# view-sonic/Cloud-Server

Hardware: AMD Instinct MI355X
Metric: train_samples_per_s (higher is better)
Workload: dtype fp32; 1 GPU; model=reference sample CNN (API.md:306-332), 2,276,218 params, global_batch=50, per_gpu_batch=50, optimizer=AdagradOptimizer, parallelism=dp1, backend=hip, hip_graph=True, collectives=none, xgmi=single rank

## Files before the change

cloud_server_amd/csrc/kernels/dense_direct.hip:

```cpp
#include "common.h"
#include "optim_common.h"
#include "head_dgrad.h"
#include <cstdlib>

namespace csa {

typedef float dd_f32x16 __attribute__((ext_vector_type(16)));

constexpr int DD_THREADS = 256;
constexpr int DD_WAVES = 4;
constexpr int DD_SLAB_ROWS = 16;
constexpr int DD_MAXC = 128;
constexpr int DD_U = 4;

__constant__ long long* g_dd_dbg = nullptr;
#define DD_STAMP(i)                                                                           \
  do {                                                                                        \
    if (g_dd_dbg && threadIdx.x == 0 && blockIdx.x == 0 && blockIdx.y == 0 && blockIdx.z == 0) \
      g_dd_dbg[i] = (long long)__builtin_amdgcn_s_memtime();                                  \
  } while (0)
#define DD_SPAN_BEGIN()                                                                       \
  do {                                                                                        \
    if (g_dd_dbg && threadIdx.x == 0)                                                         \
      atomicMin((unsigned long long*)&g_dd_dbg[4], (unsigned long long)__builtin_amdgcn_s_memtime()); \
  } while (0)
#define DD_SPAN_END()                                                                         \
  do {                                                                                        \
    if (g_dd_dbg && threadIdx.x == 0)                                                         \
      atomicMax((unsigned long long*)&g_dd_dbg[5], (unsigned long long)__builtin_amdgcn_s_memtime()); \
  } while (0)

__device__ __forceinline__ int dd_row(int r, int lane) { return (r & 3) + 8 * (r >> 2) + 4 * (lane >> 5); }

__device__ __forceinline__ void dd_pin4(float4& v) { asm volatile("" : "+v"(v.x), "+v"(v.y), "+v"(v.z), "+v"(v.w)); }
__device__ __forceinline__ void dd_pin(float& v) { asm volatile("" : "+v"(v)); }

__device__ __forceinline__ float dd_c(const float4& v, int s) {
  return s == 0 ? v.x : (s == 1 ? v.y : (s == 2 ? v.z : v.w));
}

struct DDTile { float v[8]; int row[8]; int col[8]; };

__device__ __forceinline__ DDTile dd_reduce(float* s_red, const dd_f32x16& a0, const dd_f32x16& a1) {
  const int t = threadIdx.x, lane = t & 63, w = t >> 6;
#pragma unroll
  for (int r = 0; r < 16; ++r) {
    s_red[(w * 32 + r) * 64 + lane] = a0[r];
    s_red[(w * 32 + 16 + r) * 64 + lane] = a1[r];
  }
  __syncthreads();
  DDTile out;
#pragma unroll
  for (int q = 0; q < 8; ++q) {
    const int idx = t + q * DD_THREADS;
    const int v = idx >> 6, ln = idx & 63;
    float s = s_red[(0 * 32 + v) * 64 + ln];
#pragma unroll
    for (int ww = 1; ww < DD_WAVES; ++ww) s += s_red[(ww * 32 + v) * 64 + ln];
    out.v[q] = s;
    out.row[q] = (v >> 4) * 32 + dd_row(v & 15, ln);
    out.col[q] = ln & 31;
  }
  return out;
}

__device__ __forceinline__ void dd_wave_range(int k0, int k1, int& a, int& b) {
  const int w = threadIdx.x >> 6;
  const int n8 = (k1 - k0 + 7) >> 3;
  const int per = (n8 + DD_WAVES - 1) / DD_WAVES;
  a = min(k1, k0 + w * per * 8);
  b = min(k1, a + per * 8);
}

struct DDFwd {
  const float* x; const float* w; const float* bias; float* y;
  int M, N, K, act; float alpha; int ksplit, kper;
  int life_base;
};

__constant__ long long* g_dd_life = nullptr;


template <bool V4>
__device__ __forceinline__ void dd_fwd_body(const DDFwd& a, const int nt, const int mb, const int ks, float* s_red);
// ... 384 lines not shown
      const int m = min(c0 + 2 * s + h, a.M - 1);
      xa[s] = a.x[(long)m * a.F + f];
      ya[s] = a.dy[(long)m * a.N + nc];
    }
#pragma unroll
    for (int s = 0; s < DD_KC; ++s) {
      dd_pin(xa[s]);
      dd_pin(ya[s]);
    }
#pragma unroll
    for (int s = 0; s < DD_KC; ++s) {
      if (c0 + 2 * s >= a.M) break;
      const float ok = c0 + 2 * s + h < a.M ? 1.f : 0.f;
      float xv = a.act != ACT_NONE ? act_fwd(xa[s], a.act, a.alpha) : xa[s];
      acc = __builtin_amdgcn_mfma_f32_32x32x2f32(xv * ok, ya[s], acc, 0, 0, 0);
    }
  }
  DD_STAMP(1);
  if (!upd) {
#pragma unroll
    for (int r = 0; r < 16; ++r) {
      const int ff = f0 + dd_row(r, lane);
      if (ff < a.F && nn < a.N) a.dw[(long)ff * a.N + nn] = acc[r] * a.gscale;
    }
    return;
  }
  const float lr = opt_step_lr(a.opt, a.lr, a.step);
#pragma unroll
  for (int r = 0; r < 16; ++r) {
    dd_pin(wv[r]);
    dd_pin(s0[r]);
    dd_pin(s1[r]);
  }
#pragma unroll
  for (int r = 0; r < 16; ++r) {
    const int ff = f0 + dd_row(r, lane);
    if (ff >= a.F || nn >= a.N) continue;
    const long idx = (long)ff * a.N + nn;
    opt_update(a.opt, lr, wv[r], acc[r] * a.gscale, s0[r], s1[r]);
    a.w[idx] = wv[r];
    if (ns > 0) a.sw0[idx] = s0[r];
    if (ns > 1) a.sw1[idx] = s1[r];
  }
  DD_STAMP(3);
  DD_SPAN_END();
}

constexpr int DW_WAVES = 16;
constexpr int DW_THREADS = 64 * DW_WAVES;
constexpr size_t DW_LDS = (size_t)DW_WAVES * 16 * 64 * sizeof(float);

struct DWGroup { float4 x[DD_U]; float b[DD_U][4]; };

__global__ __launch_bounds__(DW_THREADS) void dd_fwd_wide_kernel(DDFwd a, int ntile) {
  extern __shared__ __attribute__((aligned(16))) float s_part[];
  DD_STAMP(0);
  DD_SPAN_BEGIN();
  const int lb = (int)blockIdx.x, tid = threadIdx.x;
  if (g_dd_life && tid == 0) g_dd_life[2 * lb + 2 * a.life_base] = (long long)__builtin_amdgcn_s_memrealtime();
  const int lane = tid & 63, i = lane & 31, h = lane >> 5;
  const int wave = __builtin_amdgcn_readfirstlane(tid >> 6);
  const int nt = lb % ntile, ks = (lb / ntile) % a.ksplit, mb = lb / (ntile * a.ksplit);
  const int n0 = nt * 32, m0 = mb * 32;
  const int kg0 = ks * a.kper, kg1 = min(a.K, kg0 + a.kper);
  const int per = (((kg1 - kg0 + 7) >> 3) + DW_WAVES - 1) / DW_WAVES;
  const int ka = min(kg1, kg0 + wave * per * 8), kb = min(kg1, ka + per * 8);
  const float* xr = a.x + (long)min(m0 + i, a.M - 1) * a.K;
  const float* wc = a.w + min(n0 + i, a.N - 1);
  const int er = wave;
  float bias = (a.bias && ks == 0) ? a.bias[min(n0 + i, a.N - 1)] : 0.f;

  auto load = [&](DWGroup& g, int k) {
#pragma unroll
    for (int u = 0; u < DD_U; ++u) {
      if (k + 8 * u >= kb) break;
      const int kk = k + 8 * u + 4 * h;
      g.x[u] = *reinterpret_cast<const float4*>(xr + min(kk, a.K - 4));
#pragma unroll
      for (int s = 0; s < 4; ++s) g.b[u][s] = wc[(long)min(kk + s, a.K - 1) * a.N];
    }
  };
  dd_f32x16 acc = {};
  auto mac = [&](DWGroup& g, int k) {
#pragma unroll
    for (int u = 0; u < DD_U; ++u) {
      if (k + 8 * u >= kb) break;
      dd_pin4(g.x[u]);
#pragma unroll
      for (int s = 0; s < 4; ++s) dd_pin(g.b[u][s]);
      float xv[4] = {g.x[u].x, g.x[u].y, g.x[u].z, g.x[u].w};
      if (a.act != ACT_NONE) {
#pragma unroll
        for (int s = 0; s < 4; ++s) xv[s] = act_fwd(xv[s], a.act, a.alpha);
      }
      const bool in = k + 8 * u + 4 * h < kb;
#pragma unroll
      for (int s = 0; s < 4; ++s)
        acc = __builtin_amdgcn_mfma_f32_32x32x2f32(xv[s], in ? g.b[u][s] : 0.f, acc, 0, 0, 0);
    }
  };
  if (ka < kb) {
    DWGroup cur, nxt;
    load(cur, ka);
    for (int k = ka;; k += 8 * DD_U) {
      if (k + 8 * DD_U < kb) {
        load(nxt, k + 8 * DD_U);
        mac(cur, k);
        cur = nxt;
      } else {
        mac(cur, k);
        break;
      }
    }
  }
  DD_STAMP(1);
  dd_pin(bias);
#pragma unroll
  for (int r = 0; r < 16; ++r) s_part[(wave * 16 + r) * 64 + lane] = acc[r];
  __syncthreads();
  float v = bias;
  {
    const float* src = s_part + er * 64 + lane;
    float s = src[0];
#pragma unroll
    for (int w = 1; w < DW_WAVES; ++w) s += src[w * 16 * 64];
    v += s;
  }
  DD_STAMP(2);
  const int m = m0 + dd_row(er, lane), nn = n0 + i;
  if (m < a.M && nn < a.N) {
    float* p = a.y + (long)m * a.N + nn;
    if (a.ksplit > 1) atomicAdd(p, v); else *p = v;
  }
  if (g_dd_life && tid == 0) g_dd_life[2 * lb + 2 * a.life_base + 1] = (long long)__builtin_amdgcn_s_memrealtime();
  DD_STAMP(3);
  DD_SPAN_END();
}

static int dd_splits(int tiles, int K) {
  if (g_csa_det) return 1;
  static const int target = [] {
    const char* e = std::getenv("CSA_DD_TARGET");
    const int v = e ? std::atoi(e) : 2048;
    return v >= 256 && v <= 16384 ? v : 2048;
  }();
  int ks = (target / DD_WAVES + tiles - 1) / tiles;
  const int maxks = (K + 8 * DD_WAVES * 2 - 1) / (8 * DD_WAVES * 2);
  ks = ks < 1 ? 1 : ks;
  ks = ks > maxks ? maxks : ks;
  return ks < 1 ? 1 : ks;
}

static int dd_kper(int K, int ks) { return (((K + ks - 1) / ks) + 7) & ~7; }

static bool dd_wide(int K) {
  static const int wide_env = [] { const char* e = std::getenv("CSA_DD_WIDE"); return e ? (e[0] == '0' ? 0 : 1) : -1; }();
  if (wide_env == 0 || g_csa_det || g_csa_shared || (g_csa_packed && wide_env != 1)) return false;
  return K % 4 == 0;
}

struct DDPlan { bool wide; int ks, kper; };

static DDPlan dd_fwd_plan(int M, int N, int K) {
  DDPlan p;
  p.wide = dd_wide(K);
  if (p.wide) {
    static const int cap = [] { const char* e = std::getenv("CSA_DD_WIDE_KS"); return e ? std::atoi(e) : 0; }();
    const int tiles = ((N + 31) / 32) * ((M + 31) / 32);
    const int maxks = K / (8 * DW_WAVES);
    p.ks = 256 / tiles;
    p.ks = p.ks > maxks ? maxks : p.ks;
    p.ks = cap > 0 && p.ks > cap ? cap : p.ks;
    p.ks = p.ks < 1 ? 1 : p.ks;
  } else {
    p.ks = dd_splits(((N + 31) / 32) * ((M + 63) / 64), K);
  }
  p.kper = dd_kper(K, p.ks);
  p.ks = (K + p.kper - 1) / p.kper;
  return p;
}

}

using namespace csa;

CSA_API int csa_dd_life_debug(long long* p) {
  return (int)hipMemcpyToSymbol(HIP_SYMBOL(g_dd_life), &p, sizeof(p));
}

// ... 45 lines not shown
CSA_API int csa_chain_head_debug(long long* p) {
  return (int)hipMemcpyToSymbol(HIP_SYMBOL(g_hd_dbg), &p, sizeof(p));
}

static thread_local DDFwdGroup g_dd_group{};
static thread_local bool g_dd_grouping = false;
CSA_API void csa_dd_group_begin() { g_dd_grouping = true; g_dd_group.g = 0; }
CSA_API int csa_dd_group_end(hipStream_t st) {
  g_dd_grouping = false;
  const int G = g_dd_group.g;
  if (G == 0) return 0;
  const DDFwd& a0 = g_dd_group.a[0];
  for (int j = 1; j < G; ++j) {
    const DDFwd& a = g_dd_group.a[j];
    if (a.M != a0.M || a.N != a0.N || a.K != a0.K || a.ksplit != a0.ksplit || a.kper != a0.kper) return -2;
  }
  g_dd_group.ks = a0.ksplit;
  const dim3 grid((a0.N + 31) / 32, (a0.M + 63) / 64, a0.ksplit * G);
  if (a0.K % 4 == 0) hipLaunchKernelGGL(dd_fwd_group_kernel<true>, grid, dim3(DD_THREADS), 0, st, g_dd_group);
  else hipLaunchKernelGGL(dd_fwd_group_kernel<false>, grid, dim3(DD_THREADS), 0, st, g_dd_group);
  g_dd_group.g = 0;
  return (int)hipGetLastError();
}

CSA_API int csa_dd_fwd(const float* X, const float* W, const float* bias, float* Y, int M, int N, int K,
                       int act, float alpha, hipStream_t st) {
  if (M <= 0 || N <= 0 || K <= 0) return -1;
  const int nt = (N + 31) / 32, mb = (M + 63) / 64;
  const DDPlan plan = dd_fwd_plan(M, N, K);
  const int ks = plan.ks, kper = plan.kper;
  DDFwd a{X, W, bias, Y, M, N, K, act, alpha, ks, kper, 0};
  a.life_base = K > 1024 ? 0 : 4096;
  if (g_chain_on) {
    if (g_chain_n >= 2) return -4;
    g_chain_f[g_chain_n++] = a;
    return 0;
  }
  if (g_dd_grouping) {
    if (g_dd_group.g >= DD_GMAX) return -3;
    g_dd_group.a[g_dd_group.g++] = a;
    return 0;
  }
  if (plan.wide) {
    static const bool attr = hipFuncSetAttribute((const void*)dd_fwd_wide_kernel,
                                                 hipFuncAttributeMaxDynamicSharedMemorySize, (int)DW_LDS) == hipSuccess;
    (void)attr;
    const unsigned blocks = (unsigned)(nt * ((M + 31) / 32) * ks);
    hipLaunchKernelGGL(dd_fwd_wide_kernel, dim3(blocks), dim3(DW_THREADS), DW_LDS, st, a, nt);
  } else if (K % 4 == 0) hipLaunchKernelGGL(dd_fwd_kernel<true>, dim3(nt, mb, ks), dim3(DD_THREADS), 0, st, a);
  else hipLaunchKernelGGL(dd_fwd_kernel<false>, dim3(nt, mb, ks), dim3(DD_THREADS), 0, st, a);
  return (int)hipGetLastError();
}

CSA_API int csa_dd_dgrad_splits(int M, int F, int N) {
  return dd_splits(((F + 31) / 32) * ((M + 63) / 64), N);
}

CSA_API int csa_dd_dgrad_slabs() { return DD_SLAB_ROWS; }

CSA_API int csa_dd_dgrad(const float* dY, const float* W, float* dX, int M, int F, int N,
                         const float* x_fwd, int act, float alpha, const float* bn_slab, int bn_nslab, int bn_C,
                         float bn_count, float bn_eps, const float* bn_scale, const float* bn_offset,
                         float* bwd_slab, hipStream_t st) {
  if (M <= 0 || F <= 0 || N <= 0) return -1;
  if (bn_slab && (bn_C > DD_MAXC || bn_C <= 0 || !bwd_slab)) return -1;
  const int ft = (F + 31) / 32, mb = (M + 63) / 64;
  int ks = dd_splits(ft * mb, N);
  const int kper = dd_kper(N, ks);
  ks = (N + kper - 1) / kper;
  DDDgrad a{dY, W, dX, M, F, N, ks, kper, x_fwd, act, alpha,
            BNRef{bn_slab, bn_nslab, bn_C, bn_count, bn_eps, bn_scale, bn_offset}, bwd_slab};
  if (N % 4 == 0) hipLaunchKernelGGL(dd_dgrad_kernel<true>, dim3(ft, mb, ks), dim3(DD_THREADS), 0, st, a);
  else hipLaunchKernelGGL(dd_dgrad_kernel<false>, dim3(ft, mb, ks), dim3(DD_THREADS), 0, st, a);
  return (int)hipGetLastError();
}

CSA_API int csa_dd_wgrad(const float* X, const float* dY, int M, int F, int N, int act, float alpha, float gscale,
                         float* dW, float* db, float* W, float* b, float* sW0, float* sW1, float* sb0, float* sb1,
                         int opt, float lr, const int64_t* step, hipStream_t st) {
  if (M <= 0 || F <= 0 || N <= 0) return -1;
  if (opt < 0 && (!dW || !db)) return -2;
  if (opt >= 0 && (!W || !b || (opt_nslots(opt) > 0 && (!sW0 || !sb0)) || (opt_nslots(opt) > 1 && (!sW1 || !sb1))))
    return -3;
  DDWgrad a{X, dY, M, F, N, act, alpha, gscale, dW, db, W, b, sW0, sW1, sb0, sb1, opt, lr, step,
            (F + 31) / 32, (N + 127) / 128};
  const int nb = a.ftiles * a.ntiles + (N + 63) / 64;
  hipLaunchKernelGGL(dd_wgrad_kernel, dim3(nb), dim3(DD_THREADS), 0, st, a);
  return (int)hipGetLastError();
}
```

cloud_server_amd/ops/fused.py:

```python
from __future__ import annotations

import ctypes as C
import os
from typing import Optional, Sequence

import torch

from . import build as _build

_LIB: Optional[C.CDLL] = None

P = C.c_void_p
I = C.c_int
L = C.c_long
F = C.c_float
U64 = C.c_uint64

ACT_IDS = {None: 0, "none": 0, "sigmoid": 1, "relu": 2, "leaky_relu": 3}

_SIGS = {
    "csa_dense_fwd_splits": (I, [I, I, I]),
    "csa_dense_fwd": (I, [P, P, P, P, I, I, I, P, I, I, F, F, P, P, I, F, P]),
    "csa_dense_dgrad": (I, [P, P, P, I, I, I, P, I, F, P, I, I, F, F, P, P, P, P]),
    "csa_dense_dgrad_splits": (I, [I, I, I, I]),
# ... 62 lines not shown
    "csa_chain_head_debug": (I, [P]),
    "csa_dd_life_debug": (I, [P]),
    "csa_ew_life_debug": (I, [P]),
    "csa_dd_group_end": (I, [P]),
    "csa_cp_du_debug": (I, [P]),
    "csa_conv_pair_bn_tab": (None, [P]),
    "csa_conv_pair_c1_size": (L, [P]),
    "csa_conv_pair_c1_bands": (I, [P, P, I]),
    "csa_conv_pair_c1_fwd": (None, [P, L]),
    "csa_conv_pair_c1_bwd": (None, [P, L]),
    "csa_head_debug": (I, [P]),
    "csa_conv_pair_fwd": (I, [P, P, P, P, P, P, I, F, P, P, I, F, P, P, P, I, P, P, I, P]),
    "csa_conv_pair_fwd_carry": (I, [I, F, P, P, P, P, P, P, I, P, P, I]),
    "csa_opt_carry_flush": (I, [I, F, P, P, P, P, P, P, I, P, P, I, P]),
    "csa_optimizer_set_pending": (None, [P]),
    "csa_dense_update_flush_last": (I, [P]),
    "csa_conv_pair_tail_table_bytes": (L, [P, I]),
    "csa_conv_pair_tail_plan": (I, [P, I, I, P, P, P, P, P, P, P, P, I]),
    "csa_dense_update_grad_mode": (I, [P, P]),
    "csa_conv_pair_tail_set": (I, [P, P, I, F, P, P, I, I, P, P, P, P, P, P, I, L, P, P]),
    "csa_conv_pair_tail_force": (None, [P]),
    "csa_conv_pair_tail_pending": (I, []),
    "csa_conv_pair_tail_ticket_words": (I, []),
    "csa_dense_update_head_params": (I, [P, P, P, P, P, P]),
    "csa_conv_pair_valu_ok": (I, [P]),
    "csa_conv_pair_grid": (I, [P]),
    "csa_set_deterministic": (None, [I]),
    "csa_deterministic": (I, []),
    "csa_set_packed": (None, [I]),
    "csa_packed": (I, []),
    "csa_set_shared_gpu": (None, [I]),
    "csa_shared_gpu": (I, []),
    "csa_rows_fold": (I, [P, L, I, L, P, I, P]),
    "csa_rows_fold_multi": (I, [I, P, P, P, P, P, P, P]),
    "csa_conv_pair_bwd": (I, [P, P, P, P, P, P, I, F, P, I, I, F, P, P, P, P, I, F, F, P, P, P, I, P, P, P, P, F,
                              P, P, P, P, I, P, P]),
    "csa_conv_pair_bwd_tables_size": (L, [P]),
    "csa_conv_pair_bwd_tables": (I, [P, P, P]),
    "csa_conv_pair_bwd_units": (I, [P, I, P, I]),
    "csa_conv_pair_bwd_units_load": (I, [P, I, P]),
    "csa_conv_pair_bwd_bias_mode": (I, [P, I, I]),
    "csa_head_part": (I, [P, I, I, I, F, P, P, P, P, P, I, F, P, P, P, P, P, P, P]),
    "csa_head_part2": (I, [P, I, I, I, F, P, P, P, P, P, I, F, P, P, P, P, P, P, P, L, P]),
    "csa_gather_batch": (I, [P, P, P, P, I, L, P, P, P]),
    "csa_gather_images_f32": (I, [P, P, P, I, L, P, P]),
    "csa_zero": (I, [P, P, I, P]),
    "csa_gemm_debug": (I, [P]),
    "csa_conv_debug": (I, [P]),
    "csa_bn_act_apply": (I, [P, P, L, I, P, I, F, F, P, P, I, F, P, P]),
    "csa_dd_debug": (I, [P]),
    "csa_dd_fwd_splits": (I, [I, I, I]),
    "csa_dd_fwd_wide": (I, [I, I, I]),
    "csa_dd_fwd": (I, [P, P, P, P, I, I, I, I, F, P]),
    "csa_dd_dgrad_splits": (I, [I, I, I]),
    "csa_dd_dgrad_slabs": (I, []),
    "csa_dd_dgrad": (I, [P, P, P, I, I, I, P, I, F, P, I, I, F, F, P, P, P, P]),
    "csa_dd_wgrad": (I, [P, P, I, I, I, I, F, F, P, P, P, P, P, P, P, P, I, F, P, P]),
    "csa_gconv_fwd_splits": (I, [P]),
    "csa_gconv_fwd": (I, [P, P, P, P, P, P]),
    "csa_gconv_wgrad_splits": (I, [P, I]),
    "csa_gconv_wgrad": (I, [P, P, P, P, P, F, P]),
    "csa_gconv_dgrad_splits": (I, [P]),
    "csa_gconv_dgrad": (I, [P, P, P, P, P]),
    "csa_bn_slab_rows": (I, []),
    "csa_bn_stat_rows": (I, [L]),
    "csa_bn_stats": (I, [P, L, I, P, I, P]),
    "csa_bn_finalize": (I, [P, I, I, F, F, P, P, P, P, F, I, P, P]),
    "csa_bn_apply": (I, [P, P, L, I, P, I, F, P]),
    "csa_bn_bwd_reduce": (I, [P, P, P, L, I, P, I, F, P, I, P]),
    "csa_bn_bwd_finalize": (I, [P, I, I, F, F, P, P, P, P]),
    "csa_bn_bwd_apply": (I, [P, P, P, P, L, I, P, P, I, F, P]),
    "csa_maxpool_fwd": (I, [P, P, P, P, P]),
    "csa_maxpool_bwd": (I, [P, P, P, P, P]),
    "csa_drop_fwd": (I, [P, P, L, L, L, L, U64, P, P, I, F, I, F, I, P]),
    "csa_drop_bwd": (I, [P, P, P, L, L, L, L, U64, P, I, F, I, F, P]),
    "csa_xgmi_alloc":(I, [L, C.POINTER(P), P]),
    "csa_xgmi_open": (I, [P, C.POINTER(P)]),
    "csa_xgmi_reuse": (I, [P, L, P]),
    "csa_xgmi_close": (I, [P]),
    "csa_xgmi_free": (I, [P]),
    "csa_xgmi_handle_bytes": (I, []),
    "csa_xgmi_max_blocks": (I, []),
    "csa_xgmi_diag_words": (I, []),
    "csa_xgmi_run": (I, [I, I, I, L, P, P, I, P, P, P, P, C.c_double, I, P, P]),
    "csa_xgmi_reduce_scatter": (I, [I, I, L, P, P, P, L, L, L, P, P, C.c_double, I, P, P]),
    "csa_aps_step": (I, [I, I, I, I, L, I, P, P, P, P, P, P, I, F, P, P, I, C.c_double, P]),
}


def lib_path() -> str:
    return os.environ.get("CSA_KERNEL_LIB") or _build.KERNEL_LIB


def available() -> bool:
    return os.path.exists(lib_path())


def load(required: bool = True) -> Optional[C.CDLL]:
    global _LIB
    if _LIB is not None:
        return _LIB
    path = lib_path()
    if not os.path.exists(path):
        if os.environ.get("CSA_AUTOBUILD", "1") == "1":
            try:
                _build.build_kernels()
# ... 40 lines not shown
```

cloud_server_amd/runtime/hip_program.py:

```python
from __future__ import annotations

import ctypes as C
import ctypes as _ctypes
import os
from dataclasses import dataclass, field
from typing import Dict, List, Optional

import torch

from ..models.dsl import ActSpec, ConvSpec, DenseSpec, DropoutSpec, LayerPlan, NormSpec, PoolSpec
from ..ops import dropout_ref
from ..ops import fused as K
from ..ops import fused as _FK
from ..ops import optim_ref
from ..utils.streams import dedicated_stream


def _opt_call(lib, name: str, *args):
    try:
        fn = getattr(lib, name)
    except AttributeError:
        return None
    return fn(*args)

# ... 70 lines not shown
    norm: Optional[LayerPlan] = None


class HipProgram:
    WGRAD_STRIPES = int(os.environ.get("CSA_WGRAD_STRIPES", "16"))
    FWD_ZERO_MAX = 4

    def __init__(self, eng, forward_only: bool = False):
        self.e = eng
        self.forward_only = forward_only
        self.lib = K.load(required=True)
        _set_nt_out(self.lib)
        if eng.device.type != "cuda":
            raise Unsupported("HIP program needs a GPU device")
        self.det = bool(getattr(eng, "deterministic", False)) and not forward_only
        self.packed = bool(getattr(eng, "packed", False)) and os.environ.get("CSA_PACKED_PROFILE", "1") == "1"
        self.shared_gpu = bool(getattr(eng, "shared_gpu", False))
        with self._det_scope():
            self._init_plan(eng, forward_only)

    def _det_scope(self):
        prog = self

        class _Scope:
            def __enter__(self_):
                self_.prev = (int(prog.lib.csa_deterministic()), int(prog.lib.csa_packed()),
                              int(prog.lib.csa_shared_gpu()))
                prog.lib.csa_set_deterministic(1 if prog.det else 0)
                prog.lib.csa_set_packed(1 if prog.packed else 0)
                prog.lib.csa_set_shared_gpu(1 if prog.shared_gpu else 0)

            def __exit__(self_, *exc):
                prog.lib.csa_set_deterministic(self_.prev[0])
                prog.lib.csa_set_packed(self_.prev[1])
                prog.lib.csa_set_shared_gpu(self_.prev[2])
                return False
        return _Scope()

    def _init_plan(self, eng, forward_only: bool) -> None:
        self.B = eng.cfg.batch_size
        self.model = eng.model
        self.sync_bn = bool(eng.model.sync_bn)
        self.W = eng.ctx.world if self.sync_bn else 1
        self.views = eng.model.state.views(eng.flat)
        self.gviews = {} if forward_only else eng.model.state.views(eng.flat_grad)
        self._lower()
        self._plan_fused()
        self._plan_pair()
        self._plan_hfuse()
        if self.det:
            self._check_det()
        self._alloc()
        self._plan_splits()
        self.pair_tabs = None
        if self.pair is not None and not forward_only:
            n = int(self.lib.csa_conv_pair_bwd_tables_size(K.ints(self.pair)))
            if n > 0:
                self.pair_tabs = torch.zeros(n, dtype=torch.int32, device=eng.device)
                self._rc(self.lib.csa_conv_pair_bwd_tables(K.ints(self.pair), K.ptr(self.pair_tabs), K.stream()),
                         "conv_pair_bwd_tables")
        if forward_only:
            self.staged = False
            return
        self._plan_lowrank()
        self.zero_regions: List[torch.Tensor] = []
        self._collect_zero_regions()
        self._zero_now()
        self._plan_stage()
        self._plan_grad_buckets()
        self._plan_carry()
        self.opt_segments = self._opt_segments()
        self._plan_tail()
        self._plan_chain()

    def _plan_chain(self) -> None:
        e = self.e
        self.chain = False
        try:
            chain_ok = self.lib.csa_chain_ok
        except AttributeError:
            return
        dense = [u for u in self.units if u.kind == "dense"]
        if (e.ctx.enabled or self.det or self.packed or self.forward_only
                or not getattr(self, "head_dgrad", False) or os.environ.get("CSA_FWD_CHAIN", "0") != "1"
                or len(dense) != 2 or self.units[-2:] != dense or not all(u.direct for u in dense)
                or getattr(self, "br_unit", None) is not None
                or not chain_ok(self.units[-1].layer.spec.hidden)):
            return
        self.chain_tk = torch.zeros(int(self.lib.csa_chain_words()), dtype=torch.int32, device=e.device)
        self.chain_err = torch.zeros(1, dtype=torch.int32, device=e.device)
        self.chain = True

    def _plan_carry(self) -> None:
        self.carry = None
        e = self.e
        if (not e.ctx.enabled or e.sync.strategy != "allreduce" or e.aps is not None or self.pair is None
                or os.environ.get("CSA_DP_CARRY", "1") != "1"
                or not self.lib.csa_conv_pair_valu_ok(K.ints(self.pair))):
            return
        offs = self.model.state.offsets
        keep = set(self.keep_ranges)
        n = self.e.flat.numel()
        spans = sorted(offs.values())
        ends = {o: (spans[i + 1] if i + 1 < len(spans) else n) for i, o in enumerate(spans)}
        carried, segs = set(), []
        for u in self.units:
            if u.kind != "dense" or (u.fused and self.fused) or u.lr_update:
                continue
            names = [f"{u.layer.name}.weight", f"{u.layer.name}.bias"]
            if not all((offs[nm], offs[nm] + (self.gviews[nm].numel() // 4) * 4) in keep for nm in names):
                continue
            for nm in names:
                carried.add(offs[nm])
        if not carried:
            return
        for o in spans:
            if o not in carried:
                continue
            lo, hi = o - o % 4, -(-ends[o] // 4) * 4
            if segs and segs[-1][1] >= lo:
                segs[-1][1] = max(segs[-1][1], hi)
            else:
                segs.append([lo, hi])
        if len(segs) > 4:
            return
        m4 = sum(hi - lo for lo, hi in segs) // 4
        self.carry = segs
        self.carry_offsets = carried
        self.carry_blocks = max(1, min(1024, -(-m4 // 256)))
        self.carry_pending = torch.zeros(1, dtype=torch.int32, device=e.device)
        u2 = self.units[2] if len(self.units) > 2 else None
        self.carry_clear = bool(u2 is not None and u2.kind == "dense" and u2.xt is not None)

    def _carry_args(self):
        e = self.e
        s0 = e.slots[0] if e.slots.shape[0] > 0 else None
        s1 = e.slots[1] if e.slots.shape[0] > 1 else None
        lo = (C.c_long * 4)(*[x[0] for x in self.carry])
        hi = (C.c_long * 4)(*[x[1] for x in self.carry])
        return (e.opt_id, float(e.lr), K.ptr(e.dstep), K.ptr(e.flat), K.ptr(e.flat_grad), K.ptr(s0), K.ptr(s1),
                K.ptr(self.carry_pending), len(self.carry), lo, hi, self.carry_blocks)

    def flush(self, st=None) -> None:
        if getattr(self, "carry", None) is None:
# ... 541 lines not shown
                tf.count = float(B * ph * pw * self.W)
                if fo:
                    continue
                C = src.y.shape[3]
                if u.kind == "dense" and u.fused:
                    nb = self.lib.csa_dense_bwd_update_slabs(u.layer.in_shape.numel)
                elif u.kind == "dense":
                    nb = self.lib.csa_dense_dgrad_slabs(B, u.layer.in_shape.numel, u.layer.spec.hidden)
                else:
                    nb = self.lib.csa_conv_dgrad_nslab(self._conv_geom(u.layer, B))
                tf.bwd_slab = torch.zeros(nb, 2, C, **f32)
                tf.bwd_nslab = nb
                if self.det:
                    tf.bwd_prod_rows, tf.bwd_nslab = nb, 1
        for u in self.units:
            u.xt = None
            if u.kind == "dense" and u.in_tf.has_bn and u.layer.in_shape.numel % 4 == 0:
                u.xt = torch.zeros(B, u.layer.in_shape.numel, **f32)
            if u.kind == "dense" and u.fused and not fo:
                ws = (_ctypes.c_longlong * 2)()
                self.lib.csa_dense_bwd_update_ws(u.layer.in_shape.numel, u.layer.spec.hidden, ws)
                u.du_part = torch.zeros(max(int(ws[0]), 1), **f32)
                u.du_cnt = torch.zeros(max(int(ws[1]), 1), dtype=torch.int32, device=dev)
            u.in_tf.bn_tab = torch.zeros(4, u.in_tf.slab.shape[2], **f32) if u.xt is not None else None
        self.dlast = self.units[-1].dy
        if getattr(self, "head_row", False):
            self.hdl = torch.zeros(B, 10, **f32)
            self.hrl = torch.zeros(B, **f32)
            self.hrc = torch.zeros(B, dtype=torch.int32, device=dev)
        self.idx = None
        if self.head_rg:
            K = self.dlast[0].numel()
            G = -(-B // self.head_rg)
            self.head_part = torch.zeros(G, (K * 10 + 10 + 3) // 4 * 4, **f32)
            self.head_kw = K * 10
            self.head_mloss = torch.zeros(G, **f32)
            self.head_mcorr = torch.zeros(G, dtype=torch.int32, device=dev)
        self.pair_c1 = None
        if (self.pair is not None and not fo and not self.det and os.environ.get("CSA_PAIR_C1", "1") == "1"
                and self.lib.csa_conv_pair_valu_ok(_FK.ints(self.pair))):
            n = _opt_call(self.lib, "csa_conv_pair_c1_size", _FK.ints(self.pair))
            if n is not None and int(n) > 0:
                self.pair_c1 = torch.zeros(int(n), **f32)

    def _plan_splits(self) -> None:
        B = self.B
        for u in self.units:
            if u.kind == "dense":
                fin, fout = u.layer.in_shape.numel, u.layer.spec.hidden
                u.splits_fwd = (self.lib.csa_dd_fwd_splits(B, fout, fin) if u.direct
                                else self.lib.csa_dense_fwd_splits(B, fout, fin))
            elif u.kind == "gconv":
                u.splits_fwd = self.lib.csa_gconv_fwd_splits(self._conv_geom(u.layer, B))

    def _collect_zero_regions(self) -> None:
        B = self.B
        regs: List[torch.Tensor] = []
        flat: List[torch.Tensor] = []
        self.stripe_bufs: List[torch.Tensor] = []
        fold_budget = 8 - (2 if self.head_rg else 0)
        for k, u in enumerate(self.units):
            lp = u.layer
            if u.kind == "dense":
                fin, fout = lp.in_shape.numel, lp.spec.hidden
                if u.splits_fwd > 1:
                    regs.append(u.y)
                if u.fused:
                    continue
                if k > 0:
                    tfm = u.in_tf.has_bn or u.in_tf.act is not None
                    if self.lib.csa_dense_dgrad_splits(B, fin, fout, int(tfm)) > 1:
                        regs.append(self.units[k - 1].dy)
                if self.lib.csa_dense_wgrad_splits(B, fin, fout) > 1:
                    flat.append(self.gviews[f"{lp.name}.weight"].view(-1))
                    flat.append(self.gviews[f"{lp.name}.bias"])
            elif u.kind == "gconv":
                geom = self._conv_geom(lp, B)
                if u.splits_fwd > 1:
                    regs.append(u.y.view(-1))
                if k > 0 and self.lib.csa_gconv_dgrad_splits(geom) > 1:
                    regs.append(self.units[k - 1].dy.view(-1))
                if self.lib.csa_gconv_wgrad_splits(geom, int(bool(lp.spec.bias))) > 1:
                    flat.append(self.gviews[f"{lp.name}.weight"].view(-1))
                    if lp.spec.bias:
                        flat.append(self.gviews[f"{lp.name}.bias"])
            elif u.kind == "bn":
                if u.norm is not None:
                    regs += [u.bn_slab.view(-1), u.bn_bslab.view(-1)]
            elif u.kind == "conv":
                nf = 1 + (1 if lp.spec.bias else 0)
                S = 1 if self.e.ctx.enabled or fold_budget < nf else self.WGRAD_STRIPES
                in_pair = self.pair is not None and k < 2
                u.tail_fold = in_pair and getattr(self, "dp_hf", False)
                u.row_fold = self.det or (in_pair and self.e.ctx.enabled and not u.tail_fold)
                if u.tail_fold:
                    S = self.WGRAD_STRIPES
                if u.row_fold:
                    if not self.det:
                        S = self.WGRAD_STRIPES
                    elif in_pair:
                        S = int(self.lib.csa_conv_pair_grid(_FK.ints(self.pair)))
                    else:
                        S = int(self.lib.csa_conv_wgrad_blocks(self._conv_geom(lp, B), int(bool(lp.spec.bias))))
                        if S <= 0:
                            raise Unsupported(f"conv unit {lp.name}: no weight-gradient plan")
                elif S > 1:
# ... 296 lines not shown
                        K.ptr(u.dw_acc), K.ptr(u.db_acc) if sp.bias else None, u.wg_stripes, st), "conv_bwd")
                    self._conv_det_folds(u, tf, st)
                    self._grad_ready(k)
                    continue
                ws = st
                self._rc(lib.csa_conv_wgrad(
                    None if raw else K.ptr(u.x), K.ptr(img) if raw else None, K.ptr(rows) if raw else None,
                    K.ptr(dc), K.ptr(u.dw_acc), K.ptr(u.db_acc) if sp.bias else None, u.wg_stripes,
                    B, h, w, lp.in_shape.c, sp.kh, sp.kw, sp.stride[0], sp.stride[1], lp.pads[0], lp.pads[2],
                    oh, ow, sp.cout, bn[0], bn[1], bn[2], bn[3], bn[4], bn[5], in_act, in_alpha,
                    K.ptr(cur) if raw else None, ws), "conv_wgrad")
                if prev is not None:
                    self._rc(lib.csa_conv_dgrad(
                        K.ptr(dc), K.ptr(V[f"{lp.name}.weight"]), K.ptr(prev.dy), geom,
                        K.ptr(u.x), in_act, in_alpha, *bn, K.ptr(tf.bwd_slab), st), "conv_dgrad")
                self._conv_det_folds(u, tf, st)
            self._grad_ready(k)

        main = torch.cuda.current_stream(e.device)
        if e.aps is not None:
            e.aps.step(e.flat_grad, e.flat, e.slots)
            self._optimizer(st)
            return
        if self.overlap:
            main.wait_stream(self.side)
        elif e.ctx.enabled and e.sync.strategy == "lowrank":
            e.sync.allreduce_ranges(e.flat_grad, self.lr_ranges, tag="lr_rem")
            if self.lr_units:
                main.wait_stream(self.lr_side)
        else:
            e.after_backward_sync()
        if getattr(self, "tail", False):
            if lib.csa_dense_update_pending() or lib.csa_conv_pair_tail_pending():
                raise RuntimeError("pair-backward tail / deferred updates not consumed")
            if self.tail_update:
                return
        self._optimizer(st)

    _eval_bn = False

    def _forward(self, st) -> None:
        e, lib, B = self.e, self.lib, self.B
        rows, cur = e.stream.rows, e.stream.cursor
        if self.__dict__.get("x_dense_in") is not None:
            D = self.x_dense_in.shape[1]
            if e.data.images.dtype == torch.uint8 and D % 4 == 0:
                self._rc(lib.csa_gather_images_f32(K.ptr(e.data.images), K.ptr(rows), K.ptr(cur), B, D,
                                                   K.ptr(self.x_dense_in), st), "gather_images_f32")
            else:
                idx = rows.index_select(0, cur).view(-1)
                self.x_dense_in.copy_(e.data.images.index_select(0, idx).to(torch.float32).mul_(1.0 / 255.0))
        img = e.data.images
        V = self.views
        if self.pair is not None:
            ua, ub = self.units[0], self.units[1]
            nt = self.units[2].in_tf if len(self.units) > 2 else self.head_tf
            oslab = nt.slab if nt.has_bn and not self._eval_bn else None
            simg, srows, scur = self._batch_src()
            fz = [] if getattr(self, "_predicting", False) else getattr(self, "fwd_zero", [])
            carrying = getattr(self, "carry", None) is not None and not getattr(self, "_predicting", False)
            if carrying:
                self._rc(lib.csa_conv_pair_fwd_carry(*self._carry_args()), "conv_pair_fwd_carry")
            c1 = None if getattr(self, "_predicting", False) else getattr(self, "pair_c1", None)
            if c1 is not None:
                _opt_call(lib, "csa_conv_pair_c1_fwd", K.ptr(c1), c1.numel())
            self._rc(lib.csa_conv_pair_fwd(
                K.ints(self.pair), K.ptr(simg), K.ptr(srows), K.ptr(scur),
                K.ptr(V[f"{ua.layer.name}.weight"]), K.ptr(V.get(f"{ua.layer.name}.bias")) if ua.layer.spec.bias else None,
                _act_id(ua.act), _alpha(ua.act),
                K.ptr(V[f"{ub.layer.name}.weight"]), K.ptr(V.get(f"{ub.layer.name}.bias")) if ub.layer.spec.bias else None,
                _act_id(ub.act), _alpha(ub.act), K.ptr(ub.y), K.ptr(ub.argmax), K.ptr(oslab),
                nt.prod_rows if self.det else self.lib.csa_conv_fwd_nslab(None, None),
                (C.c_void_p * 4)(*[t.data_ptr() for t in fz]), (C.c_long * 4)(*[t.numel() for t in fz]), len(fz),
                st), "conv_pair_fwd")
            if carrying and self.carry_clear:
                _opt_call(lib, "csa_ew_clear_next", K.ptr(self.carry_pending))
            if oslab is not None and self.det:
                self._row_fold(oslab, nt.prod_rows, oslab.shape[1] * oslab.shape[2], oslab, 0, st)
            if oslab is not None and self.sync_bn:
                e.sync.allreduce_tensors([oslab], tag="bnf1")
        for k, u in enumerate(self.units):
            if self.pair is not None and k < 2:
                continue
            if u.kind in ("bn", "pool", "drop"):
                self._standalone_fwd(u, st)
                continue
            if u.kind == "gconv":
                self._gconv_fwd(u, st)
                continue
            lp, tf = u.layer, u.in_tf
            bn = self._bn_args(tf)
            in_act, in_alpha = _act_id(tf.act), _alpha(tf.act)
            next_tf = self.units[k + 1].in_tf if k + 1 < len(self.units) else self.head_tf
            if u.kind == "conv":
                oslab = next_tf.slab if next_tf.has_bn and not self._eval_bn else None
                raw = u.x is None
                self._rc(lib.csa_conv_fwd(
                    None if raw else K.ptr(u.x), K.ptr(img) if raw else None, K.ptr(rows) if raw else None,
                    K.ptr(V[f"{lp.name}.weight"]), K.ptr(V.get(f"{lp.name}.bias")) if lp.spec.bias else None,
                    K.ptr(u.y), K.ptr(u.argmax), K.ptr(oslab),
                    self._conv_geom(lp, B), self._pool_geom(u), *bn, in_act, in_alpha,
                    _act_id(u.act), _alpha(u.act), K.ptr(cur) if raw else None, st), "conv_fwd")
                if oslab is not None and self.det:
                    self._row_fold(oslab, next_tf.prod_rows, oslab.shape[1] * oslab.shape[2], oslab, 0, st)
                if oslab is not None and self.sync_bn:
                    e.sync.allreduce_tensors([oslab], tag=f"bnf{k}")
            else:
                fin, fout = lp.in_shape.numel, lp.spec.hidden
                if u is getattr(self, "br_unit", None):
                    self.join_branch()
                if u.xt is not None:
                    self._rc(lib.csa_bn_act_apply(
                        K.ptr(u.x), K.ptr(u.xt), B * fin, tf.slab.shape[2], *bn, in_act, in_alpha,
                        K.ptr(getattr(tf, "bn_tab", None)), st),
                        "bn_act_apply")
                if u.direct:
                    xin = u.xt if u.xt is not None else u.x.view(B, -1)
                    act = (0, 0.0) if u.xt is not None else (in_act, in_alpha)
                    self._rc(lib.csa_dd_fwd(
                        K.ptr(xin), K.ptr(V[f"{lp.name}.weight"]), K.ptr(V[f"{lp.name}.bias"]), K.ptr(u.y),
                        B, fout, fin, act[0], act[1], st), "dd_fwd")
                elif u.xt is not None:
                    self._rc(lib.csa_dense_fwd(
                        K.ptr(u.xt), K.ptr(V[f"{lp.name}.weight"]), K.ptr(V[f"{lp.name}.bias"]), K.ptr(u.y),
                        B, fout, fin, None, 0, 0, 0.0, 0.0, None, None, 0, 0.0, st), "dense_fwd")
                else:
                    self._rc(lib.csa_dense_fwd(
                        K.ptr(u.x), K.ptr(V[f"{lp.name}.weight"]), K.ptr(V[f"{lp.name}.bias"]), K.ptr(u.y),
                        B, fout, fin, *self._bn_args_c(tf), in_act, in_alpha, st), "dense_fwd")


    def _pool_geom_full(self, u: Unit):
        lp = u.layer
        sp = lp.spec
        h, w = lp.in_shape.hw
        oh, ow = lp.out_shape.hw
        return K.ints([self.B, h, w, lp.in_shape.c, sp.kernel[0], sp.kernel[1], sp.stride[0], sp.stride[1],
                       lp.pads[0], lp.pads[2], oh, ow])

    def _drop_args(self, u: Unit):
        ctx = self.e.ctx
        return (u.x.numel(), u.x[0].numel(), ctx.world, ctx.rank,
                dropout_ref.drop_seed(self.e.cfg.seed, u.layer.index))

    def _drop_consts(self, u: Unit):
        kp = u.layer.spec.keep_prob
        return (dropout_ref.keep_threshold(kp), dropout_ref.keep_scale(kp), _act_id(u.act), _alpha(u.act))

    def _standalone_fwd(self, u: Unit, st) -> None:
        lib = self.lib
        if u.kind == "drop":
            train = 0 if getattr(self, "_predicting", False) else 1
            self._rc(lib.csa_drop_fwd(K.ptr(u.x), K.ptr(u.y), *self._drop_args(u), K.ptr(self.e.dstep),
                                      K.ptr(u.used_step), *self._drop_consts(u), train, st), "drop_fwd")
            return
        if u.kind == "pool":
            self._rc(lib.csa_maxpool_fwd(K.ptr(u.x), K.ptr(u.y), K.ptr(u.argmax), self._pool_geom_full(u), st),
                     "maxpool_fwd")
            return
        n = u.x.numel()
        C_ = self._bn_channels(u)
        act, alpha = _act_id(u.act), _alpha(u.act)
        if u.norm is None:
# ... 400 lines not shown
```

Before: 788,100 samples/s.

## Fuse batch-norm stats, apply and activation into wide dense forward kernel

Adds a BN-fused variant of the wide direct-dense forward kernel. Each block reduces the BN slab statistics, computes scale and offset into LDS, and applies BN and the activation to the input tile on the fly before the MFMAs. One designated wave writes the normalized input out for the backward pass, and block 0 writes the BN table and clears the pending flag. This replaces a separate bn_act_apply launch plus a round trip of the activation through memory, at the cost of every block redundantly reducing the slab statistics. The path is enabled by default through an env flag.

```diff
diff --git a/cloud_server_amd/csrc/kernels/dense_direct.hip b/cloud_server_amd/csrc/kernels/dense_direct.hip
--- a/cloud_server_amd/csrc/kernels/dense_direct.hip
+++ b/cloud_server_amd/csrc/kernels/dense_direct.hip
@@ -30,6 +30,16 @@
       atomicMax((unsigned long long*)&g_dd_dbg[5], (unsigned long long)__builtin_amdgcn_s_memtime()); \
   } while (0)
 
+#ifdef CSA_DD_PHASES
+#define DD_PHASE(p)                                                                           \
+  do {                                                                                        \
+    if (g_dd_dbg && threadIdx.x == 0)                                                         \
+      g_dd_dbg[8 + 8 * (int)blockIdx.x + (p)] = (long long)__builtin_amdgcn_s_memrealtime();  \
+  } while (0)
+#else
+#define DD_PHASE(p) do {} while (0)
+#endif
+
 __device__ __forceinline__ int dd_row(int r, int lane) { return (r & 3) + 8 * (r >> 2) + 4 * (lane >> 5); }
 
 __device__ __forceinline__ void dd_pin4(float4& v) { asm volatile("" : "+v"(v.x), "+v"(v.y), "+v"(v.z), "+v"(v.w)); }
@@ -520,8 +530,15 @@
 
 struct DWGroup { float4 x[DD_U]; float b[DD_U][4]; };
 
-__global__ __launch_bounds__(DW_THREADS) void dd_fwd_wide_kernel(DDFwd a, int ntile) {
-  extern __shared__ __attribute__((aligned(16))) float s_part[];
+struct DDFwdBN {
+  BNRef bn; float* xt; float* tab; unsigned* clear;
+  FastDiv dc; int step8;
+};
+constexpr int DW_SU = 32;
+
+template <bool BN>
+__device__ __forceinline__ void dd_fwd_wide_body(DDFwd a, int ntile, const DDFwdBN q, float* s_part,
+                                                 float2* s_ab, float* s_mr) {
   DD_STAMP(0);
   DD_SPAN_BEGIN();
   const int lb = (int)blockIdx.x, tid = threadIdx.x;
@@ -538,6 +555,28 @@
   const int er = wave;
   float bias = (a.bias && ks == 0) ? a.bias[min(n0 + i, a.N - 1)] : 0.f;
 
+  float sv[DW_SU], ssum = 0.f, sco = 0.f;
+  int srow = 0;
+  const int C = BN ? q.bn.C : 1;
+  if constexpr (BN) {
+    if (tid < 2 * C) {
+      const int c = tid >> 1;
+      sco = (tid & 1) ? q.bn.offset[c] : q.bn.scale[c];
+      const float* col = q.bn.slab + (tid & 1) * C + c;
+      for (; srow + DW_SU < q.bn.nslab; srow += DW_SU) {
+#pragma unroll
+        for (int u = 0; u < DW_SU; ++u) sv[u] = col[(size_t)(srow + u) * 2 * C];
+#pragma unroll
+        for (int u = 0; u < DW_SU; ++u) dd_pin(sv[u]);
+#pragma unroll
+        for (int u = 0; u < DW_SU; ++u) ssum += sv[u];
+      }
+#pragma unroll
+      for (int u = 0; u < DW_SU; ++u) sv[u] = col[(size_t)min(srow + u, q.bn.nslab - 1) * 2 * C];
+    }
+    asm volatile("" ::: "memory");
+  }
+
   auto load = [&](DWGroup& g, int k) {
 #pragma unroll
     for (int u = 0; u < DD_U; ++u) {
@@ -548,6 +587,15 @@
       for (int s = 0; s < 4; ++s) g.b[u][s] = wc[(long)min(kk + s, a.K - 1) * a.N];
     }
   };
+  auto load_all = [&](DWGroup& g, int k) {
+#pragma unroll
+    for (int u = 0; u < DD_U; ++u)
+      g.x[u] = *reinterpret_cast<const float4*>(xr + min(k + 8 * u + 4 * h, a.K - 4));
+#pragma unroll
+    for (int u = 0; u < DD_U; ++u)
+#pragma unroll
+      for (int s = 0; s < 4; ++s) g.b[u][s] = wc[(long)min(k + 8 * u + 4 * h + s, a.K - 1) * a.N];
+  };
   dd_f32x16 acc = {};
   auto mac = [&](DWGroup& g, int k) {
 #pragma unroll
@@ -567,7 +615,114 @@
         acc = __builtin_amdgcn_mfma_f32_32x32x2f32(xv[s], in ? g.b[u][s] : 0.f, acc, 0, 0, 0);
     }
   };
-  if (ka < kb) {
+  int cu = 0;
+  auto mac_bn = [&](DWGroup& g, int k) {
+#pragma unroll
+    for (int u = 0; u < DD_U; ++u) dd_pin4(g.x[u]);
+    DD_PHASE(2);
+    float z[DD_U][4];
+#pragma unroll
+    for (int u = 0; u < DD_U; ++u) {
+      int c = cu;
+#pragma unroll
+      for (int s = 0; s < 4; ++s) {
+        const float2 ab = s_ab[c];
+        z[u][s] = dd_c(g.x[u], s) * ab.x + ab.y;
+        c = (c + 1 == C) ? 0 : c + 1;
+      }
+      cu += q.step8;
+      cu = cu >= C ? cu - C : cu;
+    }
+#define DD_ACT_GROUP(ACT)                                                                     \
+  _Pragma("unroll") for (int u = 0; u < DD_U; ++u)                                            \
+  _Pragma("unroll") for (int s = 0; s < 4; ++s) z[u][s] = act_fwd(z[u][s], ACT, a.alpha)
+    switch (a.act) {
+      case ACT_SIGMOID: DD_ACT_GROUP(ACT_SIGMOID); break;
+      case ACT_RELU: DD_ACT_GROUP(ACT_RELU); break;
+      case ACT_LEAKY: DD_ACT_GROUP(ACT_LEAKY); break;
+      default: break;
+    }
+#undef DD_ACT_GROUP
+#pragma unroll
+    for (int u = 0; u < DD_U; ++u) {
+      const bool in = k + 8 * u + 4 * h < kb;
+#pragma unroll
+      for (int s = 0; s < 4; ++s) dd_pin(z[u][s]);
+      g.x[u] = make_float4(in ? z[u][0] : 0.f, in ? z[u][1] : 0.f, in ? z[u][2] : 0.f, in ? z[u][3] : 0.f);
+    }
+    DD_PHASE(3);
+#ifdef CSA_DD_PHASES
+#pragma unroll
+    for (int u = 0; u < DD_U; ++u)
+#pragma unroll
+      for (int s = 0; s < 4; ++s) dd_pin(g.b[u][s]);
+    DD_PHASE(4);
+#endif
+#pragma unroll
+    for (int u = 0; u < DD_U; ++u) {
+      if (k + 8 * u >= kb) break;
+#pragma unroll
+      for (int s = 0; s < 4; ++s) dd_pin(g.b[u][s]);
+      const bool in = k + 8 * u + 4 * h < kb;
+#pragma unroll
+      for (int s = 0; s < 4; ++s)
+        acc = __builtin_amdgcn_mfma_f32_32x32x2f32(dd_c(g.x[u], s), in ? g.b[u][s] : 0.f, acc, 0, 0, 0);
+    }
+  };
+  if constexpr (BN) {
+    DWGroup cur, nxt;
+    DD_PHASE(0);
+    load_all(cur, ka);
+    if (tid < 2 * C) {
+#pragma unroll
+      for (int u = 0; u < DW_SU; ++u) dd_pin(sv[u]);
+#pragma unroll
+      for (int u = 0; u < DW_SU; ++u) ssum += srow + u < q.bn.nslab ? sv[u] : 0.f;
+    }
+    const float osum = __shfl_xor(ssum, 1, 64), oco = __shfl_xor(sco, 1, 64);
+    if (tid < 2 * C && !(tid & 1)) {
+      const int c = tid >> 1;
+      float mean = ssum / q.bn.count;
+      float var = fmaxf(osum / q.bn.count - mean * mean, 0.f);
+      float rstd = rsqrtf(var + q.bn.eps);
+      float sa = sco * rstd;
+      s_mr[c] = mean;
+      s_mr[DD_MAXC + c] = rstd;
+      s_ab[c] = make_float2(sa, oco - mean * sa);
+    }
+    __syncthreads();
+    DD_PHASE(1);
+    if (lb == 0) {
+      if (q.clear && tid == 0) *q.clear = 0u;
+      if (q.tab && tid < C) {
+        const float2 ab = s_ab[tid];
+        q.tab[tid] = s_mr[tid];
+        q.tab[C + tid] = s_mr[DD_MAXC + tid];
+        q.tab[2 * C + tid] = ab.x;
+        q.tab[3 * C + tid] = ab.y;
+      }
+    }
+    int qq;
+    q.dc.divmod(ka + 4 * h, qq, cu);
+    const bool put_ok = nt == wave % min(ntile, DW_WAVES) && m0 + i < a.M;
+    float* xo = q.xt + (long)min(m0 + i, a.M - 1) * a.K;
+    auto put = [&](DWGroup& g, int k) {
+#pragma unroll
+      for (int u = 0; u < DD_U; ++u) {
+        if (k + 8 * u >= kb) break;
+        const int kk = k + 8 * u + 4 * h;
+        if (put_ok && kk < kb) *reinterpret_cast<float4*>(xo + kk) = g.x[u];
+      }
+    };
+    for (int k = ka; k < kb; k += 8 * DD_U) {
+      const bool more = k + 8 * DD_U < kb;
+      if (more) load_all(nxt, k + 8 * DD_U);
+      mac_bn(cur, k);
+      put(cur, k);
+      DD_PHASE(5);
+      if (more) cur = nxt;
+    }
+  } else if (ka < kb) {
     DWGroup cur, nxt;
     load(cur, ka);
     for (int k = ka;; k += 8 * DD_U) {
@@ -603,6 +758,18 @@
   if (g_dd_life && tid == 0) g_dd_life[2 * lb + 2 * a.life_base + 1] = (long long)__builtin_amdgcn_s_memrealtime();
   DD_STAMP(3);
   DD_SPAN_END();
+}
+
+__global__ __launch_bounds__(DW_THREADS) void dd_fwd_wide_kernel(DDFwd a, int ntile) {
+  extern __shared__ __attribute__((aligned(16))) float s_part[];
+  dd_fwd_wide_body<false>(a, ntile, DDFwdBN{}, s_part, nullptr, nullptr);
+}
+
+__global__ __launch_bounds__(DW_THREADS) void dd_fwd_wide_bn_kernel(DDFwd a, int ntile, DDFwdBN q) {
+  extern __shared__ __attribute__((aligned(16))) float s_part[];
+  __shared__ float2 s_ab[DD_MAXC];
+  __shared__ float s_mr[2 * DD_MAXC];
+  dd_fwd_wide_body<true>(a, ntile, q, s_part, s_ab, s_mr);
 }
 
 static int dd_splits(int tiles, int K) {
@@ -754,6 +921,31 @@
   return (int)hipGetLastError();
 }
 
+CSA_API int csa_dd_fwd_bn_ok(int M, int N, int K, int C) {
+  if (M <= 0 || N <= 0 || K <= 0 || C <= 0 || C > DD_MAXC) return 0;
+  if (K % 4 != 0 || K % C != 0) return 0;
+  return dd_fwd_plan(M, N, K).wide ? 1 : 0;
+}
+
+CSA_API int csa_dd_fwd_bn(const float* X, const float* W, const float* bias, float* Y, int M, int N, int K,
+                          int C, const float* bn_slab, int bn_nslab, float bn_count, float bn_eps,
+                          const float* bn_scale, const float* bn_offset, int act, float alpha,
+                          float* xt, float* tab, unsigned* clear, hipStream_t st) {
+  if (!csa_dd_fwd_bn_ok(M, N, K, C) || !X || !xt || !bn_slab || bn_nslab <= 0 || !bn_scale || !bn_offset) return -1;
+  if (g_chain_on || g_dd_grouping) return -5;
+  const DDPlan plan = dd_fwd_plan(M, N, K);
+  DDFwd a{X, W, bias, Y, M, N, K, act, alpha, plan.ks, plan.kper, 0};
+  a.life_base = K > 1024 ? 0 : 4096;
+  DDFwdBN q{BNRef{bn_slab, bn_nslab, C, bn_count, bn_eps, bn_scale, bn_offset}, xt, tab, clear, FastDiv(C), 8 % C};
+  static const bool attr = hipFuncSetAttribute((const void*)dd_fwd_wide_bn_kernel,
+                                               hipFuncAttributeMaxDynamicSharedMemorySize, (int)DW_LDS) == hipSuccess;
+  (void)attr;
+  const int nt = (N + 31) / 32;
+  const unsigned blocks = (unsigned)(nt * ((M + 31) / 32) * plan.ks);
+  hipLaunchKernelGGL(dd_fwd_wide_bn_kernel, dim3(blocks), dim3(DW_THREADS), DW_LDS, st, a, nt, q);
+  return (int)hipGetLastError();
+}
+
 CSA_API int csa_dd_dgrad_splits(int M, int F, int N) {
   return dd_splits(((F + 31) / 32) * ((M + 63) / 64), N);
 }
diff --git a/cloud_server_amd/ops/fused.py b/cloud_server_amd/ops/fused.py
--- a/cloud_server_amd/ops/fused.py
+++ b/cloud_server_amd/ops/fused.py
@@ -138,6 +138,8 @@
     "csa_dd_fwd_splits": (I, [I, I, I]),
     "csa_dd_fwd_wide": (I, [I, I, I]),
     "csa_dd_fwd": (I, [P, P, P, P, I, I, I, I, F, P]),
+    "csa_dd_fwd_bn_ok": (I, [I, I, I, I]),
+    "csa_dd_fwd_bn": (I, [P, P, P, P, I, I, I, I, P, I, F, F, P, P, I, F, P, P, P, P]),
     "csa_dd_dgrad_splits": (I, [I, I, I]),
     "csa_dd_dgrad_slabs": (I, []),
     "csa_dd_dgrad": (I, [P, P, P, I, I, I, P, I, F, P, I, I, F, F, P, P, P, P]),
diff --git a/cloud_server_amd/runtime/hip_program.py b/cloud_server_amd/runtime/hip_program.py
--- a/cloud_server_amd/runtime/hip_program.py
+++ b/cloud_server_amd/runtime/hip_program.py
@@ -146,6 +146,7 @@
             self._check_det()
         self._alloc()
         self._plan_splits()
+        self._plan_fwd_bn()
         self.pair_tabs = None
         if self.pair is not None and not forward_only:
             n = int(self.lib.csa_conv_pair_bwd_tables_size(K.ints(self.pair)))
@@ -184,6 +185,8 @@
         self.chain_tk = torch.zeros(int(self.lib.csa_chain_words()), dtype=torch.int32, device=e.device)
         self.chain_err = torch.zeros(1, dtype=torch.int32, device=e.device)
         self.chain = True
+        for u in dense:
+            u.fwd_bn = False
 
     def _plan_carry(self) -> None:
         self.carry = None
@@ -831,6 +834,21 @@
                                 else self.lib.csa_dense_fwd_splits(B, fout, fin))
             elif u.kind == "gconv":
                 u.splits_fwd = self.lib.csa_gconv_fwd_splits(self._conv_geom(u.layer, B))
+
+    def _plan_fwd_bn(self) -> None:
+        on = os.environ.get("CSA_FWD_BN_FUSE", "1") != "0" and not self.forward_only
+        for u in self.units:
+            u.fwd_bn = False
+            if on and u.kind == "dense" and u.xt is not None and u.direct and hasattr(self.lib, "csa_dd_fwd_bn"):
+                u.fwd_bn = self._fwd_bn_ok(u)
+
+    def _fwd_bn_ok(self, u: Unit) -> bool:
+        lp = u.layer
+        return bool(_opt_call(self.lib, "csa_dd_fwd_bn_ok", self.B, lp.spec.hidden, lp.in_shape.numel,
+                              u.in_tf.slab.shape[2]))
+
+    def _fwd_bn_now(self, u: Unit) -> bool:
+        return bool(getattr(u, "fwd_bn", False)) and self._fwd_bn_ok(u)
 
     def _collect_zero_regions(self) -> None:
         B = self.B
@@ -1233,6 +1251,7 @@
                 self.x_dense_in.copy_(e.data.images.index_select(0, idx).to(torch.float32).mul_(1.0 / 255.0))
         img = e.data.images
         V = self.views
+        pend = None
         if self.pair is not None:
             ua, ub = self.units[0], self.units[1]
             nt = self.units[2].in_tf if len(self.units) > 2 else self.head_tf
@@ -1255,7 +1274,10 @@
                 (C.c_void_p * 4)(*[t.data_ptr() for t in fz]), (C.c_long * 4)(*[t.numel() for t in fz]), len(fz),
                 st), "conv_pair_fwd")
             if carrying and self.carry_clear:
-                _opt_call(lib, "csa_ew_clear_next", K.ptr(self.carry_pending))
+                if self._fwd_bn_now(self.units[2]):
+                    pend = self.carry_pending
+                else:
+                    _opt_call(lib, "csa_ew_clear_next", K.ptr(self.carry_pending))
             if oslab is not None and self.det:
                 self._row_fold(oslab, nt.prod_rows, oslab.shape[1] * oslab.shape[2], oslab, 0, st)
             if oslab is not None and self.sync_bn:
@@ -1290,6 +1312,12 @@
                 fin, fout = lp.in_shape.numel, lp.spec.hidden
                 if u is getattr(self, "br_unit", None):
                     self.join_branch()
+                if u.xt is not None and self._fwd_bn_now(u):
+                    self._rc(lib.csa_dd_fwd_bn(
+                        K.ptr(u.x), K.ptr(V[f"{lp.name}.weight"]), K.ptr(V[f"{lp.name}.bias"]), K.ptr(u.y),
+                        B, fout, fin, tf.slab.shape[2], *bn, in_act, in_alpha, K.ptr(u.xt),
+                        K.ptr(getattr(tf, "bn_tab", None)), K.ptr(pend if k == 2 else None), st), "dd_fwd_bn")
+                    continue
                 if u.xt is not None:
                     self._rc(lib.csa_bn_act_apply(
                         K.ptr(u.x), K.ptr(u.xt), B * fin, tf.slab.shape[2], *bn, in_act, in_alpha,
```

Result: faster. 803,600 samples/s (median of 6 runs) (+2.0%).
